# Vegeta2020/SE-SSD

Measured on AMD Instinct MI355X. Metric: KITTI frames/sec (voxelize->backbone->head->NMS), higher is better.
Workload: dtype f32

## Files before the change

### include/sessd_hip.h

```cpp
#ifndef SESSD_HIP_H
#define SESSD_HIP_H

#include <stddef.h>
#include <stdint.h>

#include "sessd_hip_types.h"

#ifdef __cplusplus
extern "C" {
#endif

#define SESSD_OK 0
#define SESSD_EINVAL (-1)
#define SESSD_EWORKSPACE (-2)

typedef void* sessd_stream_t;

const char* sessd_version(void);
int sessd_fill_u32(void* ptr, uint32_t value, size_t n_words, sessd_stream_t stream);
int sessd_fill_u32_multi(int n_segments, void* const* ptrs, const uint32_t* values, const size_t* n_words,
                         sessd_stream_t stream);
void sessd_set_external_clear(int on);
int sessd_stream_create_cu_mask(int n_words, const uint32_t* mask, sessd_stream_t* stream);
int sessd_stream_destroy(sessd_stream_t stream);
// ... 279 lines not shown
                    const float* shift, int relu, const float* residual, void* workspace, size_t workspace_bytes, int workgroups,
                    sessd_stream_t stream);
int sessd_conv2d_sk_active(const float* in, int batch, int cin, int hin, int win, int nclass, const float* const* wpk,
                           const int* ntaps, const int* taps_dy, const int* taps_dx, int in_mul, int tile_h, int tile_w, float* out,
                           int cout, int hout, int wout, int out_mul, const int* out_py, const int* out_px, const float* scale,
                           const float* shift, int relu, const float* residual, const int32_t* tile_list, const int32_t* n_list,
                           int list_cap, int min_rounds, void* workspace, size_t workspace_bytes, int workgroups,
                           sessd_stream_t stream);
int sessd_deconv2d_s2_mfma(const float* in, int batch, int cin, int hin, int win, const float* const* wpk4,
                           const int* ntaps4, const int* taps_dy4, const int* taps_dx4, float* out, int cout,
                           const float* scale, const float* shift, int relu, const float* residual, int tile_cfg,
                           sessd_stream_t stream);
int sessd_deconv2d_s2_mfma_pair(const float* in, int batch, int cin, int hin, int win, const float* const* wpk4_a,
                                const float* const* wpk4_b, const int* ntaps4, const int* taps_dy4, const int* taps_dx4,
                                float* out_a, float* out_b, int cout, const float* scale_a, const float* shift_a,
                                const float* scale_b, const float* shift_b, int relu, const float* residual_a,
                                const float* residual_b, int tile_cfg, sessd_stream_t stream);
int sessd_conv2d_mfma_active(const float* in, int batch, int cin, int hin, int win, const float* wpk, int ntaps, const int* taps_dy,
                             const int* taps_dx, int in_mul, int tile_h, int tile_w, float* out, int cout, int hout, int wout,
                             int out_mul, int out_py, int out_px, const float* scale, const float* shift, int relu,
                             const float* residual, const int32_t* tile_list, const int32_t* n_list, int list_cap, int tile_cfg,
                             sessd_stream_t stream);
int sessd_deconv2d_s2_mfma_pair_active(const float* in, int batch, int cin, int hin, int win, const float* const* wpk4_a,
                                       const float* const* wpk4_b, const int* ntaps4, const int* taps_dy4, const int* taps_dx4,
                                       float* out_a, float* out_b, int cout, const float* scale_a, const float* shift_a,
                                       const float* scale_b, const float* shift_b, int relu, const float* residual_a,
                                       const float* residual_b, const int32_t* tile_list, const int32_t* n_list, int list_cap,
                                       int tile_cfg, sessd_stream_t stream);
int sessd_deconv2d_s2_pair_split_active(const float* in, int batch, int cin, int hin, int win, const void* wsplit_a,
                                        const void* wsplit_b, float* out_a, float* out_b, int cout, const float* scale_a,
                                        const float* shift_a, const float* scale_b, const float* shift_b, int relu,
                                        const float* residual_a, const float* residual_b, const int32_t* tile_list,
                                        const int32_t* n_list, int list_cap, sessd_stream_t stream);
int sessd_ssfa_fuse(const float* x0, const float* x1, const float* w0, const float* w1, float bn_scale0,
                    float bn_shift0, float bn_scale1, float bn_shift1, int batch, int channels, int num_pixels,
                    float* out, sessd_stream_t stream);
int sessd_nchw_split_nhwc(const float* planar, int batch, int channels, int plane, int n_parts, const int* sizes,
                          float* const* parts, sessd_stream_t stream);
int sessd_nhwc_merge_nchw(float* const* parts, int n_parts, const int* sizes, int batch, int channels, int plane, float* planar,
                          sessd_stream_t stream);
size_t sessd_ssfa_fuse_train_workspace_bytes(int batch, int channels, int plane);
int sessd_ssfa_fuse_train_fwd(const float* x0, const float* x1, int batch, int channels, int plane, const float* w0,
                              const float* w1, const float* gamma0, const float* beta0, const float* gamma1, const float* beta1,
                              float eps, float momentum, float* running_mean0, float* running_var0, float* running_mean1,
                              float* running_var1, float* out, float* smap, float* stats, void* workspace,
                              size_t workspace_bytes, sessd_stream_t stream);
int sessd_ssfa_fuse_train_bwd(const float* grad_out, const float* x0, const float* x1, int batch, int channels, int plane,
                              const float* w0, const float* w1, const float* gamma0, const float* beta0, const float* gamma1,
                              const float* beta1, const float* smap, const float* stats, float* dzmap, float* dx0, float* dx1,
                              float* dw0, float* dw1, float* dgamma, float* dbeta, void* workspace, size_t workspace_bytes,
                              sessd_stream_t stream);
int sessd_ssfa_fuse_head(const float* x0, const float* x1, const float* w0, const float* w1, float bn_scale0, float bn_shift0,
                         float bn_scale1, float bn_shift1, int batch, int channels, int num_pixels, float* out,
                         const float* head_w, const float* head_b, int nout, float* head_out, sessd_stream_t stream);
int sessd_ssfa_fuse_head_keys(const float* x0, const float* x1, const float* w0, const float* w1, float bn_scale0,
                              float bn_shift0, float bn_scale1, float bn_shift1, int batch, int channels, int num_pixels,
                              float* out, const float* head_w, const float* head_b, int nout, float* head_out,
                              float score_thresh, unsigned long long* keys, int key_cap, int32_t* key_count,
                              sessd_stream_t stream);
int sessd_ssfa_fuse_head_tasks(const float* x0, const float* x1, const float* w0, const float* w1, float bn_scale0,
                               float bn_shift0, float bn_scale1, float bn_shift1, int batch, int channels, int num_pixels,
                               float* out, const float* head_w, const float* head_b, int num_tasks, float* head_out,
                               float score_thresh, unsigned long long* keys, int key_cap, int32_t* key_count,
                               sessd_stream_t stream);
int sessd_rpn_up_head_tasks(const float* x, const float* up_w, const float* up_scale, const float* up_shift, int batch,
                            int channels, int num_pixels, float* out, const float* head_w, const float* head_b, int num_tasks,
// ... 53 lines not shown
```

### se-ssd_amd/sessd_hip/_lib.py

```python
import ctypes as C
import os

import torch

_HERE = os.path.dirname(os.path.abspath(__file__))
LIB_PATH = os.path.join(os.path.dirname(_HERE), "lib", "libsessd_hip.so")

vp, i32, u32, f32, sz, i64, f64 = C.c_void_p, C.c_int, C.c_uint32, C.c_float, C.c_size_t, C.c_longlong, C.c_double



class ChainLevel(C.Structure):
    _fields_ = [("ksize", i32 * 3), ("stride", i32 * 3), ("pad", i32 * 3), ("out_dims", i32 * 3), ("cap", i32),
                ("indices", vp), ("n_dev", vp)]


class RulebookJob(C.Structure):
    _fields_ = [("in_level", i32), ("out_level", i32), ("ksize", i32 * 3), ("stride", i32 * 3), ("pad", i32 * 3),
                ("nbr", vp), ("tile_mask", vp), ("site_mask", vp), ("perm", vp), ("tile_mask_sorted", vp)]


class FillTilesJob(C.Structure):
    _fields_ = [("out", vp), ("value", vp), ("tile_mask", vp), ("cout", i32), ("h", i32), ("w", i32), ("mask_th", i32), ("tile", i32),
                ("near_kind", i32), ("near_mask", vp)]
# ... 59 lines not shown
    "sessd_boxes_pairwise": (i32, [i32, vp, i32, vp, i32, vp, vp]),
    "sessd_boxes_aligned_overlap_bev": (i32, [vp, vp, i32, vp, vp]),
    "sessd_rotate_iou_eval": (i32, [vp, i32, vp, i32, i32, vp, vp]),
    "sessd_box3d_overlap_eval": (i32, [vp, i32, vp, i32, i32, i32, f64, vp, vp]),
    "sessd_kitti_statistics": (i32, [vp, vp, vp, vp, vp, vp, vp, vp, vp, vp, i32, i32, f64, vp, i32, i32, i32, vp, vp, vp, vp]),
    "sessd_kitti_reduce": (i32, [vp, i32, i32, vp, vp]),
    "sessd_kitti_thresholds": (i32, [vp, i32, i32, i32, vp, vp, vp]),
    "sessd_nms_workspace_bytes": (sz, [i32]),
    "sessd_nms_sorted": (i32, [i32, vp, i32, f32, vp, vp, vp, sz, vp]),
    "sessd_nms_axis_eps_sorted": (i32, [vp, i32, i32, f32, f32, vp, vp, vp, sz, vp]),
    "sessd_conv2d_mfma": (i32, [vp, i32, i32, i32, i32, vp, i32, vp, vp, i32, i32, i32, vp, i32, i32, i32, i32, i32, i32,
                                vp, vp, i32, vp, i32, vp]),
    "sessd_conv3x3_winograd": (i32, [vp, i32, i32, i32, i32, vp, vp, i32, vp, vp, i32, vp, i32, vp]),
    "sessd_conv2d_pack_taps": (i32, [vp, i64, i64, vp, i32, i32, i32, vp, vp]),
    "sessd_conv3x3_winograd_pack": (i32, [vp, i64, i64, i32, i32, i32, i32, vp, vp]),
    "sessd_conv3x3_winograd_sk_workspace_bytes": (sz, [i32, i32, i32, i32, i32, i32]),
    "sessd_conv3x3_winograd_sk_sets": (i32, [vp, i32, i32, i32, i32, i32, vp, vp, i32, vp, vp, i32, vp, vp, sz, i32, i32, vp]),
    "sessd_conv3x3_winograd_sk": (i32, [vp, i32, i32, i32, i32, vp, vp, i32, vp, vp, i32, vp, vp, sz, i32, i32, vp]),
    "sessd_conv3x3_winograd_sk_active": (i32, [vp, i32, i32, i32, i32, vp, vp, i32, vp, vp, i32, vp, vp, vp, i32, i32, vp, sz, i32, i32, vp]),
    "sessd_bev_tile_activity_workspace_bytes": (sz, [i32, i32]),
    "sessd_bev_tile_activity": (i32, [vp, vp, i32, i32, i32, i32, vp, i32, vp, vp, vp, i32, vp, sz, vp]),
    "sessd_fill_inactive_tiles": (i32, [vp, i32, i32, vp]),
    "sessd_conv2d_sk_workspace_bytes": (sz, [i32, i32, i32, i32, i32, i32]),
    "sessd_conv2d_sk_pack": (i32, [vp, i64, i64, vp, i32, i32, i32, vp, vp]),
    "sessd_conv2d_sk": (i32, [vp, i32, i32, i32, i32, i32, vp, vp, vp, vp, i32, i32, i32, vp, i32, i32, i32, i32, vp, vp, vp, vp,
                              i32, vp, vp, sz, i32, vp]),
    "sessd_conv2d_sk_active": (i32, [vp, i32, i32, i32, i32, i32, vp, vp, vp, vp, i32, i32, i32, vp, i32, i32, i32, i32, vp, vp, vp, vp,
                                     i32, vp, vp, vp, i32, i32, vp, sz, i32, vp]),
    "sessd_conv2d_mfma_active": (i32, [vp, i32, i32, i32, i32, vp, i32, vp, vp, i32, i32, i32, vp, i32, i32, i32, i32, i32, i32, vp, vp, i32, vp,
                                       vp, vp, i32, i32, vp]),
    "sessd_deconv2d_s2_mfma_pair_active": (i32, [vp, i32, i32, i32, i32, vp, vp, vp, vp, vp, vp, vp, i32, vp, vp, vp, vp, i32, vp, vp, vp, vp,
                                                 i32, i32, vp]),
    "sessd_deconv2d_s2_pair_split_active": (i32, [vp, i32, i32, i32, i32, vp, vp, vp, vp, i32, vp, vp, vp, vp, i32, vp, vp, vp, vp, i32, vp]),
    "sessd_deconv2d_s2_mfma_pair": (i32, [vp, i32, i32, i32, i32, vp, vp, vp, vp, vp, vp, vp, i32, vp, vp, vp, vp, i32, vp, vp, i32, vp]),
    "sessd_deconv2d_s2_mfma": (i32, [vp, i32, i32, i32, i32, vp, vp, vp, vp, vp, i32, vp, vp, i32, vp, i32, vp]),
    "sessd_ssfa_fuse": (i32, [vp, vp, vp, vp, f32, f32, f32, f32, i32, i32, i32, vp, vp]),
    "sessd_ssfa_fuse_head": (i32, [vp, vp, vp, vp, f32, f32, f32, f32, i32, i32, i32, vp, vp, vp, i32, vp, vp]),
    "sessd_predict_workspace_bytes": (sz, [i32, i32, i32, i32]),
    "sessd_predict": (i32, [vp, i32, i32, vp, i32, vp, f32, i32, i32, f32, vp, f32, vp, vp, vp, vp, vp, sz, vp]),
    "sessd_predict_fused": (i32, [vp, i32, i32, vp, i32, vp, f32, i32, i32, f32, vp, f32, vp, vp, vp, vp, vp, vp, vp, vp, i32, vp, vp, sz, vp]),
    "sessd_ssfa_fuse_head_keys": (i32, [vp, vp, vp, vp, f32, f32, f32, f32, i32, i32, i32, vp, vp, vp, i32, vp, f32, vp, i32, vp, vp]),
    "sessd_ssfa_fuse_head_tasks": (i32, [vp, vp, vp, vp, f32, f32, f32, f32, i32, i32, i32, vp, vp, vp, i32, vp, f32, vp, i32, vp, vp]),
    "sessd_rpn_up_head_tasks": (i32, [vp, vp, vp, vp, i32, i32, i32, vp, vp, vp, i32, vp, f32, vp, i32, vp, vp]),
    "sessd_predict_tasks_workspace_bytes": (sz, [i32, i32, i32, i32, i32]),
    "sessd_predict_tasks": (i32, [vp, i32, i32, i32, vp, i32, vp, f32, i32, i32, f32, vp, f32, vp, vp, vp, vp, vp, vp, vp, vp, vp, i32, vp, vp,
                                  sz, vp]),
    "sessd_predict_di_workspace_bytes": (sz, [i32, i32, i32, i32, i32]),
    "sessd_predict_di": (i32, [vp, i32, i32, i32, vp, i32, vp, f32, i32, i32, f32, vp, f32, vp, vp, vp, vp, vp, vp, vp, vp, vp, i32, vp, vp,
                               vp, vp, vp, vp, vp, sz, vp]),
    "sessd_di_nms_workspace_bytes": (sz, [i32]),
    "sessd_di_nms": (i32, [vp, vp, vp, i32, vp, vp, vp, vp, vp, i32, f32, vp, i32, vp, f32, i32, vp, vp, vp, vp, vp, vp, vp, sz, vp]),
    "sessd_pack_detections": (i32, [vp, vp, vp, vp, i32, i32, vp, vp, i32, vp, vp]),
    "sessd_quads_pairwise": (i32, [i32, vp, i32, vp, i32, vp, f32, vp, vp]),
    "sessd_rotate_nms_workspace_bytes": (sz, [i32]),
    "sessd_rotate_nms_sorted": (i32, [vp, i32, f32, i32, vp, vp, vp, sz, vp]),
    "sessd_rotate_nms_corners_sorted": (i32, [vp, i32, f32, i32, vp, vp, vp, sz, vp]),
    "sessd_sparse_hash_build": (i32, [vp, vp, i32, vp, vp, vp, u32, vp]),
    "sessd_sparse_downsample_workspace_bytes": (sz, [i32, i32, u32]),
    "sessd_sparse_downsample_sites": (i32, [vp, vp, i32, vp, vp, vp, vp, vp, vp, u32, vp, i32, vp, vp, vp, sz, vp]),
    "sessd_sparse_rulebook": (i32, [vp, vp, i32, vp, vp, vp, vp, vp, u32, vp, vp, vp, vp]),
    "sessd_sparse_rulebook_pair": (i32, [vp, vp, i32, vp, vp, vp, vp, vp, u32, vp, vp, vp, vp, vp, vp, vp, vp, u32, vp, vp, vp, vp]),
    "sessd_sparse_downsample_sites_unordered": (i32, [vp, vp, i32, vp, vp, vp, vp, vp, vp, u32, vp, i32, vp, vp, vp]),
    "sessd_sparse_to_dense": (i32, [vp, vp, i32, i32, vp, vp, vp]),
    "sessd_dense_to_sparse": (i32, [vp, vp, i32, i32, vp, vp, vp]),
    "sessd_sparse_to_dense_dev": (i32, [vp, vp, i32, vp, i32, vp, vp, vp]),
    "sessd_dense_to_sparse_dev": (i32, [vp, vp, i32, vp, i32, vp, vp, vp]),
# ... 76 lines not shown
```

### se-ssd_amd/sessd_hip/engine.py

```python
import math
import os

import numpy as np
import torch

from ._lib import lib, check
from . import ops


def _round_up(v, m):
    return (int(v) + m - 1) // m * m


def fold_bn(bn):
    w = bn.weight.detach().float() if bn.weight is not None else torch.ones_like(bn.running_mean)
    b = bn.bias.detach().float() if bn.bias is not None else torch.zeros_like(bn.running_mean)
    scale = w / torch.sqrt(bn.running_var.detach().float() + bn.eps)
    shift = b - bn.running_mean.detach().float() * scale
    return scale.contiguous(), shift.contiguous()


WINO_SPLIT = os.environ.get("SESSD_WINO_SPLIT", "1") != "0"
WINO_LIST_SHAPES = (0, 1, 3) if WINO_SPLIT else (0, 1)
DECONV_SPLIT = os.environ.get("SESSD_DECONV_SPLIT", "1") != "0"
PAIR_SPLIT_CFG = 45

SPMIDDLE_LAYERS = [
    ("subm", 4, 16, 3, 1, 0, "subm0"), ("subm", 16, 16, 3, 1, 0, "subm0"),
    ("conv", 16, 32, 3, 2, 1, None),
    ("subm", 32, 32, 3, 1, 0, "subm1"), ("subm", 32, 32, 3, 1, 0, "subm1"),
    ("conv", 32, 64, 3, 2, 1, None),
    ("subm", 64, 64, 3, 1, 0, "subm2"), ("subm", 64, 64, 3, 1, 0, "subm2"), ("subm", 64, 64, 3, 1, 0, "subm2"),
    ("conv", 64, 64, 3, 2, [0, 1, 1], None),
    ("subm", 64, 64, 3, 1, 0, "subm3"), ("subm", 64, 64, 3, 1, 0, "subm3"), ("subm", 64, 64, 3, 1, 0, "subm3"),
    ("conv", 64, 64, (3, 1, 1), (2, 1, 1), 0, None),
]


def _t3(v):
    return [int(v)] * 3 if isinstance(v, int) else [int(x) for x in v]


class SparsePlan:

    def __init__(self, convs, bns, layers, device):
        self.layers = []
        for (kind, cin, cout, ks, st, pd, key), conv, bn in zip(layers, convs, bns):
            w = conv.weight.detach().to(device=device, dtype=torch.float32).contiguous()
            assert tuple(w.shape[-2:]) == (cin, cout), (w.shape, cin, cout)
            scale, shift = fold_bn(bn)
            self.layers.append(dict(kind=kind, cin=cin, cout=cout, ks=_t3(ks), st=_t3(st), pd=_t3(pd), key=key,
                                    wpk=ops.sparse_pack_weight(w), scale=scale.to(device), shift=shift.to(device)))


def active_tile_constants(neck):
    b0, b1 = neck.bottom_up_block_0, neck.bottom_up_block_1
    def step(seq, ci, bi, c):
        s_, t_ = fold_bn(seq[bi])
# ... 449 lines not shown
        for l in ids:
            if l in (self.ACTIVE_PAIR, self.ACTIVE_CONV):
                for o, v in zip(self.ACTIVE_SLOTS[l][3], self.dn.act_const[l]):
                    outs.append(o); vals.append(v); slots.append(self.ACTIVE_MASK[l]); tiles.append(4 if l == self.ACTIVE_PAIR else 6)
                    near.append(None); kinds.append(0)
                continue
            nr, kind = None, 0
            if self.near_fill:
                rd = self.NEAR_READER.get(l)
                if rd is not None and rd in ids and rd not in self.ACTIVE_SK:
                    nr = self.ACTIVE_MASK[rd]
                elif self.form != "ssfa":
                    pass
                elif self.coarse_fill and l == 2 and 3 in ids and 6 in ids:
                    nr, kind = self.ACTIVE_MASK[3], 2
                elif self.coarse_fill and l == 6 and self.ACTIVE_PAIR in ids:
                    nr, kind = self.ACTIVE_MASK[self.ACTIVE_PAIR], 1
                elif self.coarse_fill and l == 5 and 7 in ids:
                    continue
            outs.append(self.ACTIVE_SLOTS[l][3]); vals.append(self.dn.act_const[l]); slots.append(self.ACTIVE_MASK[l]); tiles.append(2)
            near.append(nr); kinds.append(kind)
        return outs, vals, slots, tiles, near, kinds

    def _active_layers(self):
        if self.ta is None or self._tuning is not None or self.sk_ws is None:
            return []
        return sorted(self.active_cfg)

    def _conv(self, x, layer, out, relu=True, residual=None, name=None, active=None):
        pc, scale, shift = layer
        if active is not None:
            shape, min_rounds = self.active_cfg[active]
            m = self.ACTIVE_MASK[active]
            if active in self.ACTIVE_SK and shape != 30:
                call = lambda: ops.conv2d_mfma_active(x, pc, scale, shift, relu, out, self.ta.tile_list[m], self.ta.n_list[m:m + 1],
                                                      tile_cfg=shape, residual=residual)
            elif active in self.ACTIVE_SK:
                call = lambda: ops.conv2d_sk_active(x, pc, scale, shift, relu, out, self.sk_ws, self.ta.tile_list[m],
                                                    self.ta.n_list[m:m + 1], workgroups=self._wgs(2), residual=residual,
                                                    min_rounds=min_rounds)
            else:
                call = lambda: ops.conv2d_winograd_sk_active(x, pc.upk_sk(shape), pc.cout, scale, shift, relu, out, shape, self.sk_ws,
                                                             self.ta.tile_list[m], self.ta.n_list[m:m + 1],
                                                             workgroups=self._wgs(shape), residual=residual, min_rounds=min_rounds)
            if self._kmarks is not None:
                e0, e1 = torch.cuda.Event(enable_timing=True), torch.cuda.Event(enable_timing=True)
                e0.record()
                r = call()
                e1.record()
                self._kmarks.append((name, e0, e1))
                return r
            return call()
        if self._tuning is not None:
            self._tuning.append((name, x, layer, out, relu, residual))
        if self._kmarks is not None:
            e0, e1 = torch.cuda.Event(enable_timing=True), torch.cuda.Event(enable_timing=True)
            e0.record()
            r = ops.conv2d(x, pc, scale, shift, relu, residual, out, self.tile_cfg.get(name), workspace=self.sk_ws, workgroups=self._wgs_cfg(self.tile_cfg.get(name)))
            e1.record()
            self._kmarks.append((name, e0, e1))
            return r
        return ops.conv2d(x, pc, scale, shift, relu, residual, out, self.tile_cfg.get(name), workspace=self.sk_ws, workgroups=self._wgs_cfg(self.tile_cfg.get(name)))

    def adopt_tuning(self, other):
        self.tile_cfg = dict(other.tile_cfg)
        self.active_cfg = dict(other.active_cfg) if self.ta is not None else {}
        self.sparse_split = dict(other.sparse_split)
        self.sparse_sorted = dict(other.sparse_sorted)
        self.sk_workgroups = other.sk_workgroups
        self.cu_budget = other.cu_budget
        self.merge_branch_convs = other.merge_branch_convs
        self.sk_ws = torch.zeros_like(other.sk_ws) if other.sk_ws is not None else None

    DEFAULT_ACTIVE_CFG = {0: (1, 4), 1: (0, 1), 2: (1, 2), 3: (30, 4), 4: (1, 2), 5: (0, 1), 6: (11, 0), 7: (30, 8), 8: (4, 0), 9: (0, 8)}
    if WINO_SPLIT:
        DEFAULT_ACTIVE_CFG = {l: ((3, mr) if shape == 0 else (shape, mr)) for l, (shape, mr) in DEFAULT_ACTIVE_CFG.items()}

    def force_active_tiles(self, active_cfg=None):
        if self.ta is None:
            raise RuntimeError("this engine has no tile-activity program (active_tiles=False or an unsupported BEV size)")
        if self.form == "rpn":
            self.tile_cfg.update({"blk0.%d" % i: 22 for i in range(len(self.dn.layers))})
            self._need_sk_ws(max(int(lib.sessd_conv3x3_winograd_sk_workspace_bytes(self.B, self.H, self.W, 128, sh, 0)) for sh in (0, 1)))
            cfg = dict(self.DEFAULT_ACTIVE_CFG if active_cfg is None else active_cfg)
            for l, (shape, mr) in cfg.items():
                if l not in self.ACTIVE_SLOTS:
                    raise ValueError("an RPN engine's list layers are %s, got %r" % (sorted(self.ACTIVE_SLOTS), l))
                if self.ACTIVE_SLOTS[l][1][0].upk_sk(shape) is None:
                    raise ValueError("active-tile layer %s: no stream-K Winograd packing for shape %d" % (self.ACTIVE_SLOTS[l][0], shape))
            self.active_cfg = cfg
            return self.active_cfg
        self.tile_cfg.update({"b0.0": 22, "b0.1": 22, "b0.2": 23, "b1.0": 30, "b1.1": 23, "b1.2": 22, "trans_0": 30, "trans_1": 30,
                              "conv_0": 22, "conv_1": 22})
        B = self.B
        self._need_sk_ws(max([int(lib.sessd_conv3x3_winograd_sk_workspace_bytes(2 * B, self.H, self.W, 256, sh, 0)) for sh in (0, 1)] +
                             [int(lib.sessd_conv2d_sk_workspace_bytes(B, self.H, self.W, 256, 1, 0))]))
        cfg = dict(self.DEFAULT_ACTIVE_CFG if active_cfg is None else active_cfg)
        for l, (shape, mr) in cfg.items():
            if l == self.ACTIVE_PAIR and shape == PAIR_SPLIT_CFG and any(pc.wsplit() is None for pc, _, _ in self.ACTIVE_SLOTS[l][1]):
                raise ValueError("active-tile layer %s: no split weight planes (cin %% 16)" % self.ACTIVE_SLOTS[l][0])
            if l in self.ACTIVE_SK or l == self.ACTIVE_PAIR:
                continue
            layers = self.ACTIVE_SLOTS[l][1] if l == self.ACTIVE_CONV else (self.ACTIVE_SLOTS[l][1],)
            if any(pc.upk_sk(shape) is None for pc, _, _ in layers):
                raise ValueError("active-tile layer %s: no stream-K Winograd packing for shape %d" % (self.ACTIVE_SLOTS[l][0], shape))
        self.active_cfg = cfg
        return self.active_cfg

    def autotune(self, candidates=(1, 2, 3, 4, 6, 11, 12), reps=5):
        self._tuning, self._tuning_sparse = [], []
        self.enqueue()
        torch.cuda.synchronize()
        todo, self._tuning = self._tuning, None
        todo_sp, self._tuning_sparse = self._tuning_sparse, None
        st = torch.cuda.current_stream().cuda_stream
        for idx, lay, in_feat, nbr, tm, out_li, out_feat in todo_sp:
            best = (None, 1e30)
            cands = [(a, b, c) for c in ((0, 1) if self.allow_offset_split else (0,)) for a in (1, 2, 4) for b in (2, 3, 4)]
            cands += [(a, 2, 2) for a in (1, 2, 4)]
            if self.levels[out_li]["cap"] >= 65536 or getattr(self, "sparse_mt_candidates", False):
                cands += [(a, b, c) for c in (16, 32) for a in (1, 2, 4) for b in (2, 3)]
            for split, depth, ks in cands:
                if (lay["cout"] // 16) % split or (ks == 1 and depth == 4):
                    continue
                for srt in ((True, False) if self.chain.sort_tiles else (False,)):
                    self.sparse_split[idx] = split + 256 * depth + 65536 * ks
                    self.sparse_sorted[idx] = srt
                    for _ in range(2):
                        self._sconv(lay, in_feat, nbr, tm, out_li, out_feat, st, idx=idx)
                    e0, e1 = torch.cuda.Event(enable_timing=True), torch.cuda.Event(enable_timing=True)
                    e0.record()
                    for _ in range(reps):
                        self._sconv(lay, in_feat, nbr, tm, out_li, out_feat, st, idx=idx)
                    e1.record()
                    torch.cuda.synchronize()
                    t = e0.elapsed_time(e1) / reps
# ... 108 lines not shown
                    dense_t = self.tune_report.get("conv_0", (None, 0.0))[1] + self.tune_report.get("conv_1", (None, 0.0))[1]
                for shape in WINO_LIST_SHAPES:
                    if p0.upk_sk(shape) is None or p1.upk_sk(shape) is None:
                        continue
                    self._need_sk_ws(int(lib.sessd_conv3x3_winograd_sk_workspace_bytes(self.B, self.H, self.W, p0.cout, shape, 0)))
                    for mr in (4, 8, 16, -1):
                        def both(shape=shape, mr=mr):
                            for (pc_, sc_, sh_), xi, xo in ((layer[0], x_in[0], x_out[0]), (layer[1], x_in[1], x_out[1])):
                                ops.conv2d_winograd_sk_active(xi, pc_.upk_sk(shape), pc_.cout, sc_, sh_, True, xo, shape, self.sk_ws,
                                                              self.ta.tile_list[m], self.ta.n_list[m:m + 1], workgroups=self._wgs(shape), min_rounds=mr)
                        tt = timed(both)
                        if tt < best[1]:
                            best = ((shape, mr), tt)
                special_dense[l] = dense_t
                if best[0] is not None and best[1] < dense_t:
                    pick[l] = best
                    gain += dense_t - best[1]
                continue
            pc, scale, shift = layer
            if l in self.ACTIVE_SK:
                if pc.launches[0].ntaps == 1 and pc.cin % 8 == 0:
                    for cfg in (3, 4, 11, 12):
                        tt = timed(lambda: ops.conv2d_mfma_active(x_in, pc, scale, shift, True, x_out, self.ta.tile_list[m],
                                                                  self.ta.n_list[m:m + 1], tile_cfg=cfg))
                        if tt < best[1]:
                            best = ((cfg, 0), tt)
                if pc.sk_args() is not None:
                    self._need_sk_ws(int(lib.sessd_conv2d_sk_workspace_bytes(self.B, *pc.tile_hw(*x_in.shape[2:]), pc.cout, len(pc.launches), 0)))
                    for mr in (1, 4, 8, 16):
                        tt = timed(lambda: ops.conv2d_sk_active(x_in, pc, scale, shift, True, x_out, self.sk_ws, self.ta.tile_list[m],
                                                                self.ta.n_list[m:m + 1], workgroups=self._wgs(2), min_rounds=mr))
                        if tt < best[1]:
                            best = ((30, mr), tt)
            else:
                for shape in WINO_LIST_SHAPES:
                    if pc.upk_sk(shape) is None:
                        continue
                    self._need_sk_ws(int(lib.sessd_conv3x3_winograd_sk_workspace_bytes(self.B, x_in.shape[2], x_in.shape[3], pc.cout, shape, 0)))
                    for mr in self.list_share_candidates:
                        tt = timed(lambda: ops.conv2d_winograd_sk_active(x_in, pc.upk_sk(shape), pc.cout, scale, shift, True, x_out, shape,
                                                                         self.sk_ws, self.ta.tile_list[m], self.ta.n_list[m:m + 1],
                                                                         workgroups=self._wgs(shape), min_rounds=mr))
                        if tt < best[1]:
                            best = ((shape, mr), tt)
            dense_t = self.tune_report.get(name, (None, 0.0))[1]
            if best[0] is not None and best[1] < dense_t:
                pick[l] = best
                gain += dense_t - best[1]
        def overhead(ids):
            fj = self._fill_jobs(ids)
            return timed(lambda: (self.ta.run(L4["indices"], L4["n"], L4["cap"]), self.ta.fill(fj[0], fj[1], layers=fj[2], tiles=fj[3], near=fj[4], near_kind=fj[5])),
                         4 * reps)
        sl = sorted(pick)
        over = overhead(sl) if pick else 0.0
        for l in (self.ACTIVE_CONV, self.ACTIVE_PAIR, 7, 6):
            if l in pick and len(pick) > 1:
                rest = [q for q in sl if q != l]
                over_wo = overhead(rest)
                g = (special_dense[l] if l in special_dense else
                     self.tune_report.get(self.ACTIVE_SLOTS[l][0], (None, 0.0))[1] if l != self.ACTIVE_PAIR else pair_dense_t) - pick[l][1]
                if over - over_wo >= g:
                    del pick[l]
                    sl, over, gain = rest, over_wo, gain - g
        if pick and gain > over:
            self.active_cfg = {l: pick[l][0] for l in pick}
        self.tune_report["active_tiles"] = ({self.ACTIVE_SLOTS[l][0]: v for l, v in self.active_cfg.items()}, gain - over, over,
# ... 436 lines not shown
```

### se-ssd_amd/sessd_hip/ops.py

```python
import ctypes
import os

import torch

from ._lib import lib, check, SessdError


def _stream():
    return torch.cuda.current_stream().cuda_stream


def _p(t):
    return 0 if t is None else t.data_ptr()


def _addr(arr):
    return ctypes.cast(arr, ctypes.c_void_p).value


def _req(t, dtype, name):
    if not t.is_cuda:
        raise ValueError("%s must be a CUDA (HIP) tensor: the SE-SSD hot path has no CPU fallback" % name)
    if t.dtype != dtype:
        raise TypeError("%s must be %s, got %s" % (name, dtype, t.dtype))
# ... 1356 lines not shown
    ws = torch.empty(int(lib.sessd_sparse_conv_wgrad_workspace_bytes(kv, cin, cout)), dtype=torch.uint8, device=in_feat.device)
    check(lib.sessd_sparse_conv_wgrad(in_feat.data_ptr(), cin, grad_out.data_ptr(), cout, nbr.data_ptr(), tile_mask.data_ptr(),
                                      kv, n_out_dev.data_ptr(), cap, gw.data_ptr(), ws.data_ptr(), ws.numel(), _stream()),
          "sparse_conv_wgrad")
    return gw


class Launch:
    __slots__ = ("dy", "dx", "in_mul", "out_mul", "py", "px", "ntaps", "view", "_wpk", "_owner")

    def __init__(self, dy, dx, in_mul, out_mul, py, px, view):
        self.dy, self.dx, self.in_mul, self.out_mul, self.py, self.px, self.view = dy, dx, in_mul, out_mul, py, px, view
        self.ntaps = len(view[3])
        self._wpk = self._owner = None

    @property
    def wpk(self):
        if self._wpk is None:
            pc = self._owner
            self._wpk = pc._make(lambda: _pack_taps_view(*self.view, pc.cout, pc.cin))
        return self._wpk


class PackedConv:

    def __init__(self, launches, cin, cout, kind, stride, w3=None, wt=None):
        self.launches = launches
        self.cin, self.cout, self.kind, self.stride = cin, cout, kind, stride
        self._w3, self._wt = w3, wt
        self._upk = None
        self._upk_sk = [None, None, None, None]
        self._sk = None
        self._wsplit = None
        self._registry = None
        for la in launches:
            la._owner = self
        self.wpk4 = self.ntaps4 = self.dy4 = self.dx4 = None
        if wt is not None:
            self.wpk4 = (ctypes.c_void_p * 4)(*[la.wpk.data_ptr() for la in launches])
            self.ntaps4 = torch.tensor([la.ntaps for la in launches], dtype=torch.int32)
            self.dy4 = torch.zeros((4, 4), dtype=torch.int32)
            self.dx4 = torch.zeros((4, 4), dtype=torch.int32)
            for c, la in enumerate(launches):
                self.dy4[c, :la.ntaps] = la.dy
                self.dx4[c, :la.ntaps] = la.dx

    def _make(self, make):
        return self._registry.create(make) if self._registry is not None else make()

    def out_hw(self, H, W):
        s = self.stride
        return ((H + s - 1) // s, (W + s - 1) // s) if self.kind == "conv" else (s * H, s * W)

    def tile_hw(self, H, W):
        return self.out_hw(H, W) if self.kind == "conv" else (H, W)

    @property
    def is_3x3_s1(self):
        return self._w3 is not None

    @property
    def upk(self):
        if self._upk is None and self.is_3x3_s1 and self.cin % 8 == 0:
            self._upk = self._make(lambda: pack_winograd(self._w3[0], adjoint=self._w3[1]))
        return self._upk

    def upk_sk(self, shape):
        if self._upk_sk[shape] is None and self.is_3x3_s1 and self.cin % (16, 8, 16, 16)[shape] == 0:
            self._upk_sk[shape] = self._make(lambda: pack_winograd_sk(self._w3[0], shape, adjoint=self._w3[1]))
        return self._upk_sk[shape]

    def wsplit(self):
        if self._wt is None or self.cin % 16:
            return None
        if self._registry is not None:
            return pack_deconv2d_s2_split(self._wt)
        if self._wsplit is None:
            self._wsplit = pack_deconv2d_s2_split(self._wt)
        return self._wsplit

    def sk_args(self):
        if self._sk is None:
            n = len(self.launches)
            if self.cin % 16 or n > 4:
                return None
            ncg = (self.cout + 127) // 128
            wpk, dy, dx = [], (ctypes.c_int * (9 * n))(), (ctypes.c_int * (9 * n))()
            for c, la in enumerate(self.launches):
                w, so, sc, taps = la.view
                nt = len(taps)
                out = torch.empty((ncg, self.cin // 16, nt, 2048), dtype=torch.float32, device=w.device)
                check(lib.sessd_conv2d_sk_pack(w.data_ptr(), int(so), int(sc), (ctypes.c_int * nt)(*[int(t) for t in taps]), nt,
                                               self.cout, self.cin, out.data_ptr(), _stream()), "conv2d_sk_pack")
                wpk.append(out)
                for t in range(nt):
                    dy[9 * c + t], dx[9 * c + t] = int(la.dy[t]), int(la.dx[t])
            self._sk = dict(wpk=wpk, wptr=(ctypes.c_void_p * n)(*[t.data_ptr() for t in wpk]),
                            ntaps=(ctypes.c_int * n)(*[la.ntaps for la in self.launches]), dy=dy, dx=dx,
                            py=(ctypes.c_int * n)(*[la.py for la in self.launches]),
                            px=(ctypes.c_int * n)(*[la.px for la in self.launches]), n=n)
        return self._sk


def _pack_taps_view(w, out_stride, in_stride, tap_offsets, cout, cin):
    _req(w, torch.float32, "weight")
    nt = len(tap_offsets)
    cp = (cout + 31) // 32 * 32
    out = torch.empty((cin // 2, nt, 2, cp), dtype=torch.float32, device=w.device)
    check(lib.sessd_conv2d_pack_taps(w.data_ptr(), int(out_stride), int(in_stride), (ctypes.c_int * nt)(*[int(t) for t in tap_offsets]),
                                     nt, cout, cin, out.data_ptr(), _stream()), "conv2d_pack_taps")
    _repack_note("dense", w=w, out=out, so=int(out_stride), sc=int(in_stride), taps=[int(t) for t in tap_offsets], cout=int(cout),
                 cin=int(cin), kind=0, flip=0, layout=0)
# ... 244 lines not shown

DECONV_SPLIT_TAPS = ((1, 1), (1, 2), (2, 1), (2, 2), (1, 0), (2, 0), (0, 1), (0, 2), (0, 0))


def pack_deconv2d_s2_split(weight):
    w = weight.detach().to(torch.float32)
    ci, co, kh, kw = w.shape
    if kh != 3 or kw != 3 or ci % 16:
        raise ValueError("pack_deconv2d_s2_split: a (Cin, Cout, 3, 3) weight with Cin % 16 == 0")
    ng = (co + 127) // 128
    wt = torch.zeros((9, ci, ng * 128), dtype=torch.float32, device=w.device)
    for t, (ky, kx) in enumerate(DECONV_SPLIT_TAPS):
        wt[t, :, :co] = w[:, :, ky, kx]
    planes = []
    for _ in range(3):
        p = wt.to(torch.bfloat16)
        planes.append(p)
        wt = wt - p.to(torch.float32)
    pl = torch.stack(planes).view(3, 9, ci // 16, 2, 8, ng, 4, 32)
    return pl.permute(5, 2, 1, 0, 6, 3, 7, 4).contiguous().view(ng, ci // 16, 9, 3, 4, 64, 8)


def deconv2d_s2_pair_split_active(x, pc_a, pc_b, scale_a, shift_a, scale_b, shift_b, relu, out_a, out_b, tile_list, n_list, residual_a=None,
                                  residual_b=None):
    _req(tile_list, torch.int32, "tile_list"); _req(n_list, torch.int32, "n_list")
    wa, wb = pc_a.wsplit(), pc_b.wsplit()
    if wa is None or wb is None:
        raise ValueError("deconv2d_s2_pair_split_active needs cin % 16 == 0")
    args = _pair_args(x, pc_a, pc_b, (wa.data_ptr(), wb.data_ptr()), scale_a, shift_a, scale_b, shift_b, relu, out_a, out_b, residual_a,
                      residual_b)
    check(lib.sessd_deconv2d_s2_pair_split_active(*args, tile_list.data_ptr(), n_list.data_ptr(), tile_list.numel(), _stream()),
          "deconv2d_s2_pair_split_active")
    return out_a, out_b


def pack_deconv2d_ks(weight, s):
    w = weight.detach().to(torch.float32).contiguous()
    ci, co, kh, kw = w.shape
    s = int(s)
    assert s >= 2 and kh == s and kw == s and ci % 2 == 0
    zero = torch.zeros(1, dtype=torch.int32)
    launches = []
    for py in range(s):
        for px in range(s):
            launches.append(Launch(zero, zero, 1, s, py, px, (w, s * s, co * s * s, [py * s + px])))
    pc = PackedConv(launches, ci, co, "deconv_ks", s)
    for la in launches:
        la.wpk
    return pc


class PackedDeconvKs:

    def __init__(self, wpk, cin, cout, s):
        self.wpk, self.cin, self.cout, self.stride, self.kind = wpk, cin, cout, s, "deconv_ks_slice"


def pack_deconv_ks_slice(weight, s):
    w = weight.detach().to(torch.float32).contiguous()
    _req(w, torch.float32, "weight")
    ci, co, kh, kw = w.shape
    s = int(s)
    if s not in (1, 2, 4) or kh != s or kw != s:
        raise ValueError("pack_deconv_ks_slice: kernel size = stride in {1, 2, 4} expected, got kernel %dx%d, s = %d" % (kh, kw, s))
    if ci % 2 or co % 32:
        raise ValueError("pack_deconv_ks_slice: even cin and cout %% 32 == 0 expected, got %d -> %d" % (ci, co))
# ... 700 lines not shown
```

Before: 2236.

## Add bf16x3-split MFMA kernel for active-tile 3x3 stride-2 conv

Adds a new HIP kernel for the active-tile 3x3 stride-2 BEV conv. It splits f32 activations and weights into three bf16 planes and accumulates the cross terms with 32x32x16 bf16 MFMA, using double-buffered LDS and a pipeline tuned with scheduling barriers. The autotuner now times this path against the existing stream-K and MFMA variants and selects it only when it is fastest. The bf16x3 split aims for near-f32 accuracy through bf16 matrix cores, at the cost of extra MFMAs and a separate weight packing.

Result: faster. 2284 (median of 6 runs) (+2.1%).

```diff
diff --git a/include/sessd_hip.h b/include/sessd_hip.h
--- a/include/sessd_hip.h
+++ b/include/sessd_hip.h
@@ -335,6 +335,9 @@
                                         const float* shift_a, const float* scale_b, const float* shift_b, int relu,
                                         const float* residual_a, const float* residual_b, const int32_t* tile_list,
                                         const int32_t* n_list, int list_cap, sessd_stream_t stream);
+int sessd_conv2d_s2_split_active(const float* in, int batch, int cin, int hin, int win, const void* wsplit, float* out, int cout,
+                                 int hout, int wout, const float* scale, const float* shift, int relu, const float* residual,
+                                 const int32_t* tile_list, const int32_t* n_list, int list_cap, sessd_stream_t stream);
 int sessd_ssfa_fuse(const float* x0, const float* x1, const float* w0, const float* w1, float bn_scale0,
                     float bn_shift0, float bn_scale1, float bn_shift1, int batch, int channels, int num_pixels,
                     float* out, sessd_stream_t stream);
diff --git a/se-ssd_amd/csrc/dense_conv_s2_split.hip b/se-ssd_amd/csrc/dense_conv_s2_split.hip
--- /dev/null
+++ b/se-ssd_amd/csrc/dense_conv_s2_split.hip
@@ -0,0 +1,273 @@
+#include "common.hpp"
+#include "bf16_split.hpp"
+
+namespace {
+
+using f32x16 = __attribute__((ext_vector_type(16))) float;
+typedef unsigned int u32x2g __attribute__((__vector_size__(8)));
+typedef unsigned int u32x4g __attribute__((__vector_size__(16)));
+typedef __bf16 bf16x8 __attribute__((ext_vector_type(8)));
+using sessd::split3_pk;
+
+typedef __amdgpu_buffer_rsrc_t rsrc_t;
+__device__ __forceinline__ rsrc_t make_rsrc(const void* base, unsigned bytes) {
+  return __builtin_amdgcn_make_buffer_rsrc(const_cast<void*>(base), (short)0, (int)bytes, 0x00020000);
+}
+__device__ __forceinline__ float bufload(rsrc_t rsrc, unsigned voff, unsigned soff) {
+  return __builtin_bit_cast(float, __builtin_amdgcn_raw_buffer_load_b32(rsrc, (int)voff, (int)soff, 0));
+}
+#define SESSD_OOB 0x80000000u
+#define SESSD_LDS_BARRIER() asm volatile("s_waitcnt lgkmcnt(0)\n\ts_barrier" ::: "memory")
+
+struct ConvS2SplitArgs {
+  const float* in;
+  const void* w;
+  float* out;
+  const float* scale;
+  const float* shift;
+  const float* residual;
+  const int* tile_list;
+  const int* n_list;
+  int list_cap, batch, cin, hin, win, cout, hout, wout, relu, ngroups;
+};
+
+__device__ __forceinline__ bool tile_of(const ConvS2SplitArgs& A, int n_list, int k, int& img, int& y0, int& x0) {
+  const int ntiles2 = (A.hout >> 1) * (A.wout >> 1), tw2 = A.wout >> 1;
+  const int ent = k < n_list ? A.tile_list[k] : -1;
+  const bool live = ent >= 0 && ent < A.batch * ntiles2;
+  img = live ? ent / ntiles2 : 0;
+  const int t = live ? ent - img * ntiles2 : 0;
+  y0 = 2 * (t / tw2);
+  x0 = 2 * (t - (t / tw2) * tw2);
+  return live;
+}
+
+constexpr int XBUF = 3 * 2 * 3 * 256;
+
+__global__ __launch_bounds__(256, 2) void conv_s2_split_kernel(ConvS2SplitArgs A) {
+  __shared__ __attribute__((aligned(16))) unsigned lds[2 * XBUF];
+  const int tid = threadIdx.x, lane = tid & 63, wave = tid >> 6;
+  const int j = lane & 31, h = lane >> 5;
+  const int n_list = __builtin_amdgcn_readfirstlane(min(A.n_list[0], A.list_cap));
+  const int unit = blockIdx.x / A.ngroups, grp = blockIdx.x - unit * A.ngroups;
+  if (unit * 16 >= n_list) return;
+
+  const int npix = A.hin * A.win;
+  const unsigned plane4 = (unsigned)npix * 4u;
+  const int KS = A.cin >> 4;
+  const rsrc_t xr = make_rsrc(A.in, (unsigned)A.batch * A.cin * plane4);
+  const rsrc_t wr = make_rsrc(A.w, (unsigned)A.ngroups * KS * (27u * 4096u));
+
+  const int spb = wave & 1, sq = wave >> 1;
+  unsigned xo[3][3];
+  {
+    int img, y0, x0;
+    const bool live = tile_of(A, n_list, unit * 16 + spb * 8 + (j >> 2), img, y0, x0);
+    const int iy0 = 2 * (y0 + ((j >> 1) & 1)) - 1, ix0 = 2 * (x0 + (j & 1)) - 1;
+    const unsigned base = (unsigned)(img * A.cin + h * 8 + sq * 4) * (unsigned)npix;
+#pragma unroll
+    for (int ky = 0; ky < 3; ++ky)
+#pragma unroll
+      for (int kx = 0; kx < 3; ++kx) {
+        const int iy = iy0 + ky, ix = ix0 + kx;
+        xo[ky][kx] = (live && iy >= 0 && iy < A.hin && ix >= 0 && ix < A.win) ? (base + (unsigned)(iy * A.win + ix)) * 4u : SESSD_OOB;
+      }
+  }
+  const int wthr = (spb * 3 * 64 + lane) * 4 + sq * 2;
+  float xs[3][4];
+#define SESSD_CS_LOADX(KSTEP, KY)                                                                   \
+  {                                                                                                 \
+    const unsigned c0 = (unsigned)min((KSTEP), KS - 1) * 16u;                                       \
+    _Pragma("unroll") for (int kx = 0; kx < 3; ++kx)                                                \
+      _Pragma("unroll") for (int i = 0; i < 4; ++i)                                                 \
+        xs[kx][i] = bufload(xr, xo[KY][kx], (c0 + i) * plane4);                                     \
+  }
+#define SESSD_CS_SPLIT_STORE(VOFF)                                                                  \
+  {                                                                                                 \
+    _Pragma("unroll") for (int kx = 0; kx < 3; ++kx) {                                              \
+      u32x2g t0, t1, t2;                                                                            \
+      _Pragma("unroll") for (int q = 0; q < 2; ++q) {                                               \
+        unsigned a0, a1, a2;                                                                        \
+        split3_pk(xs[kx][2 * q], xs[kx][2 * q + 1], a0, a1, a2);                                    \
+        t0[q] = a0; t1[q] = a1; t2[q] = a2;                                                         \
+      }                                                                                             \
+      unsigned* dst = lds + (VOFF) + wthr + kx * (2 * 3 * 256);                                     \
+      *static_cast<u32x2g*>(__builtin_assume_aligned(dst, 8)) = t0;                                 \
+      *static_cast<u32x2g*>(__builtin_assume_aligned(dst + 256, 8)) = t1;                           \
+      *static_cast<u32x2g*>(__builtin_assume_aligned(dst + 512, 8)) = t2;                           \
+    }                                                                                               \
+  }
+
+  const int cb = wave;
+  const int rthr = lane * 4;
+  const unsigned wvo = (unsigned)(cb * 1024 + lane * 16);
+  const unsigned wgrp = (unsigned)grp * (unsigned)KS * (27u * 4096u);
+  const int tlast = KS * 9 - 1;
+  f32x16 acc[2], accl[2], tot[2];
+  const f32x16 zero16 = {0.f, 0.f, 0.f, 0.f, 0.f, 0.f, 0.f, 0.f, 0.f, 0.f, 0.f, 0.f, 0.f, 0.f, 0.f, 0.f};
+#pragma unroll
+  for (int q = 0; q < 2; ++q) acc[q] = accl[q] = tot[q] = zero16;
+  bf16x8 af[3][3], bf[2][2][3];
+
+#define SESSD_CS_LOADA(SET, TG)                                                                     \
+  {                                                                                                 \
+    const unsigned ws = wgrp + (unsigned)min((TG), tlast) * (3u * 4096u);                           \
+    _Pragma("unroll") for (int p = 0; p < 3; ++p)                                                   \
+      af[SET][p] = __builtin_bit_cast(bf16x8, __builtin_amdgcn_raw_buffer_load_b128(wr, (int)wvo, (int)(ws + 4096u * p), 0)); \
+  }
+#define SESSD_CS_READB(VOFF, KX, BS)                                                                \
+  {                                                                                                 \
+    _Pragma("unroll") for (int q = 0; q < 2; ++q)                                                   \
+      _Pragma("unroll") for (int p = 0; p < 3; ++p)                                                 \
+        bf[BS][q][p] = __builtin_bit_cast(bf16x8, *static_cast<const u32x4g*>(__builtin_assume_aligned( \
+            lds + (VOFF) + rthr + (((KX)*2 + q) * 3 + p) * 256, 16)));                              \
+  }
+#define SESSD_CS_M(ACC, KX, BS, PA, PB)                                                             \
+  _Pragma("unroll") for (int q = 0; q < 2; ++q)                                                     \
+    ACC[q] = __builtin_amdgcn_mfma_f32_32x32x16_bf16(af[KX][PA], bf[BS][q][PB], ACC[q], 0, 0, 0);
+#define SESSD_CS_MSMALL(KX, BS)                                                                     \
+  SESSD_CS_M(accl, KX, BS, 2, 0)                                                                    \
+  SESSD_CS_M(accl, KX, BS, 1, 1)                                                                    \
+  SESSD_CS_M(accl, KX, BS, 0, 2)                                                                    \
+  SESSD_CS_M(accl, KX, BS, 1, 0)                                                                    \
+  SESSD_CS_M(accl, KX, BS, 0, 1)
+#define SESSD_CS_MMA(KX, BS)                                                                        \
+  {                                                                                                 \
+    SESSD_CS_MSMALL(KX, BS)                                                                         \
+    SESSD_CS_M(acc, KX, BS, 0, 0)                                                                   \
+  }
+#define SESSD_CS_MMA_FIRST(BS)                                                                      \
+  {                                                                                                 \
+    _Pragma("unroll") for (int q = 0; q < 2; ++q) tot[q] += acc[q];                                 \
+    SESSD_CS_MSMALL(0, BS)                                                                          \
+    _Pragma("unroll") for (int q = 0; q < 2; ++q)                                                   \
+      acc[q] = __builtin_amdgcn_mfma_f32_32x32x16_bf16(af[0][0], bf[BS][q][0], zero16, 0, 0, 0);    \
+  }
+#define SESSD_CS_STEP(KS_, KY, S0, S1)                                                              \
+  {                                                                                                 \
+    const int tg = (KS_)*9 + (KY)*3;                                                                \
+    SESSD_CS_READB(voff, 1, S1)                                                                     \
+    SESSD_CS_LOADA(2, tg + 2)                                                                       \
+    __builtin_amdgcn_sched_barrier(0);                                                              \
+    SESSD_CS_MMA_FIRST(S0)                                                                          \
+    SESSD_CS_SPLIT_STORE(voff ^ XBUF)                                                               \
+    _Pragma("unroll") for (int g = 0; g < 12; ++g) {                                                \
+      __builtin_amdgcn_sched_group_barrier(0x008, 1, 0);                                            \
+      __builtin_amdgcn_sched_group_barrier(0x002, 9, 0);                                            \
+    }                                                                                               \
+    __builtin_amdgcn_sched_barrier(0);                                                              \
+    SESSD_CS_READB(voff, 2, S0)                                                                     \
+    SESSD_CS_LOADX((KS_) + ((KY) + 2) / 3, ((KY) + 2) % 3)                                          \
+    SESSD_CS_LOADA(0, tg + 3)                                                                       \
+    __builtin_amdgcn_sched_barrier(0);                                                              \
+    SESSD_CS_MMA(1, S1)                                                                             \
+    __builtin_amdgcn_sched_barrier(0);                                                              \
+    SESSD_LDS_BARRIER();                                                                            \
+    voff ^= XBUF;                                                                                   \
+    SESSD_CS_READB(voff, 0, S1)                                                                     \
+    SESSD_CS_LOADA(1, tg + 4)                                                                       \
+    __builtin_amdgcn_sched_barrier(0);                                                              \
+    SESSD_CS_MMA(2, S0)                                                                             \
+    __builtin_amdgcn_sched_barrier(0);                                                              \
+  }
+
+  int voff = 0;
+  SESSD_CS_LOADX(0, 0)
+  SESSD_CS_LOADA(0, 0)
+  SESSD_CS_LOADA(1, 1)
+  __builtin_amdgcn_sched_barrier(0);
+  SESSD_CS_SPLIT_STORE(0)
+  SESSD_CS_LOADX(0, 1)
+  SESSD_LDS_BARRIER();
+  SESSD_CS_READB(0, 0, 0)
+  __builtin_amdgcn_sched_barrier(0);
+  int ks = 0;
+  for (; ks + 1 < KS; ks += 2) {
+    SESSD_CS_STEP(ks, 0, 0, 1)
+    SESSD_CS_STEP(ks, 1, 1, 0)
+    SESSD_CS_STEP(ks, 2, 0, 1)
+    SESSD_CS_STEP(ks + 1, 0, 1, 0)
+    SESSD_CS_STEP(ks + 1, 1, 0, 1)
+    SESSD_CS_STEP(ks + 1, 2, 1, 0)
+  }
+  if (ks < KS) {
+    SESSD_CS_STEP(ks, 0, 0, 1)
+    SESSD_CS_STEP(ks, 1, 1, 0)
+    SESSD_CS_STEP(ks, 2, 0, 1)
+  }
+#undef SESSD_CS_LOADX
+#undef SESSD_CS_SPLIT_STORE
+#undef SESSD_CS_LOADA
+#undef SESSD_CS_READB
+#undef SESSD_CS_M
+#undef SESSD_CS_MMA
+#undef SESSD_CS_MSMALL
+#undef SESSD_CS_MMA_FIRST
+#undef SESSD_CS_STEP
+
+  const unsigned oplane = (unsigned)(A.hout * A.wout);
+  const unsigned obytes = (unsigned)A.batch * A.cout * oplane * 4u;
+  const float* res = A.residual;
+  const rsrc_t orr = make_rsrc(A.out, obytes);
+  const rsrc_t rr = make_rsrc(res ? res : A.out, res ? obytes : 0u);
+  const rsrc_t scr = make_rsrc(A.scale ? A.scale : A.in, A.scale ? (unsigned)A.cout * 4u : 0u);
+  const rsrc_t shr = make_rsrc(A.shift ? A.shift : A.in, A.shift ? (unsigned)A.cout * 4u : 0u);
+  const int co0 = grp * 128 + cb * 32 + 4 * h;
+  float scv[16], shv[16];
+#pragma unroll
+  for (int r = 0; r < 16; ++r) {
+    const int k = (r & 3) + 8 * (r >> 2);
+    scv[r] = A.scale ? bufload(scr, (unsigned)(co0 + k) * 4u, 0) : 1.f;
+    shv[r] = bufload(shr, (unsigned)(co0 + k) * 4u, 0);
+  }
+#pragma unroll
+  for (int q = 0; q < 2; ++q) {
+    int img, y0, x0;
+    const bool live = tile_of(A, n_list, unit * 16 + q * 8 + (j >> 2), img, y0, x0);
+    const int y = y0 + ((j >> 1) & 1), x = x0 + (j & 1);
+    const unsigned vbase = ((unsigned)(img * A.cout + co0) * oplane + (unsigned)(y * A.wout + x)) * 4u;
+    unsigned vo[16];
+    float rv[16];
+#pragma unroll
+    for (int r = 0; r < 16; ++r) {
+      const int k = (r & 3) + 8 * (r >> 2);
+      vo[r] = (live && co0 + k < A.cout) ? vbase + (unsigned)k * oplane * 4u : SESSD_OOB;
+      rv[r] = bufload(rr, vo[r], 0);
+    }
+#pragma unroll
+    for (int r = 0; r < 16; ++r) {
+      float v = fmaf((tot[q][r] + acc[q][r]) + accl[q][r], scv[r], shv[r]);
+      if (A.relu) v = fmaxf(v, 0.f);
+      if (res) v += rv[r];
+      __builtin_amdgcn_raw_buffer_store_b32(__builtin_bit_cast(unsigned, v), orr, (int)vo[r], 0, 0);
+    }
+  }
+}
+
+size_t split_pack_bytes(int cin, int cout) { return (size_t)sessd_divup(cout, 128) * (cin / 16) * 27 * 4096; }
+
+}
+
+extern "C" {
+
+int sessd_conv2d_s2_split_active(const float* in, int batch, int cin, int hin, int win, const void* wsplit, float* out, int cout,
+                                 int hout, int wout, const float* scale, const float* shift, int relu, const float* residual,
+                                 const int32_t* tile_list, const int32_t* n_list, int list_cap, hipStream_t stream) {
+  if (cin < 16 || cin % 16 || batch < 1 || cout < 1 || hout < 2 || wout < 2 || (hout & 1) || (wout & 1)) return SESSD_EINVAL;
+  if ((hin != 2 * hout && hin != 2 * hout - 1) || (win != 2 * wout && win != 2 * wout - 1)) return SESSD_EINVAL;
+  if (!in || !wsplit || !out || !tile_list || !n_list || list_cap < 1) return SESSD_EINVAL;
+  if ((long long)batch * cout * hout * wout * 4 >= 0x7fffffffLL || (long long)batch * cin * hin * win * 4 >= 0x7fffffffLL) return SESSD_EINVAL;
+  if (split_pack_bytes(cin, cout) >= 0x7fffffffULL) return SESSD_EINVAL;
+  ConvS2SplitArgs A;
+  A.in = in; A.w = wsplit; A.out = out; A.scale = scale; A.shift = shift; A.residual = residual;
+  A.tile_list = tile_list; A.n_list = n_list; A.list_cap = list_cap;
+  A.batch = batch; A.cin = cin; A.hin = hin; A.win = win; A.cout = cout; A.hout = hout; A.wout = wout; A.relu = relu;
+  A.ngroups = sessd_divup(cout, 128);
+  const long long wgs = (long long)sessd_divup(list_cap, 16) * A.ngroups;
+  if (wgs > 0x7fffffffLL) return SESSD_EINVAL;
+  SESSD_LAUNCH(conv_s2_split_kernel, dim3((unsigned)wgs), dim3(256), 0, stream, A);
+  SESSD_CHECK_LAUNCH();
+  return SESSD_OK;
+}
+
+}
diff --git a/se-ssd_amd/sessd_hip/_lib.py b/se-ssd_amd/sessd_hip/_lib.py
--- a/se-ssd_amd/sessd_hip/_lib.py
+++ b/se-ssd_amd/sessd_hip/_lib.py
@@ -115,6 +115,7 @@
     "sessd_deconv2d_s2_mfma_pair_active": (i32, [vp, i32, i32, i32, i32, vp, vp, vp, vp, vp, vp, vp, i32, vp, vp, vp, vp, i32, vp, vp, vp, vp,
                                                  i32, i32, vp]),
     "sessd_deconv2d_s2_pair_split_active": (i32, [vp, i32, i32, i32, i32, vp, vp, vp, vp, i32, vp, vp, vp, vp, i32, vp, vp, vp, vp, i32, vp]),
+    "sessd_conv2d_s2_split_active": (i32, [vp, i32, i32, i32, i32, vp, vp, i32, i32, i32, vp, vp, i32, vp, vp, vp, i32, vp]),
     "sessd_deconv2d_s2_mfma_pair": (i32, [vp, i32, i32, i32, i32, vp, vp, vp, vp, vp, vp, vp, i32, vp, vp, vp, vp, i32, vp, vp, i32, vp]),
     "sessd_deconv2d_s2_mfma": (i32, [vp, i32, i32, i32, i32, vp, vp, vp, vp, vp, i32, vp, vp, i32, vp, i32, vp]),
     "sessd_ssfa_fuse": (i32, [vp, vp, vp, vp, f32, f32, f32, f32, i32, i32, i32, vp, vp]),
diff --git a/se-ssd_amd/sessd_hip/engine.py b/se-ssd_amd/sessd_hip/engine.py
--- a/se-ssd_amd/sessd_hip/engine.py
+++ b/se-ssd_amd/sessd_hip/engine.py
@@ -24,6 +24,8 @@
 WINO_LIST_SHAPES = (0, 1, 3) if WINO_SPLIT else (0, 1)
 DECONV_SPLIT = os.environ.get("SESSD_DECONV_SPLIT", "1") != "0"
 PAIR_SPLIT_CFG = 45
+CONV_S2_SPLIT = os.environ.get("SESSD_CONV_S2_SPLIT", "1") != "0"
+S2_SPLIT_CFG = 46
 
 SPMIDDLE_LAYERS = [
     ("subm", 4, 16, 3, 1, 0, "subm0"), ("subm", 16, 16, 3, 1, 0, "subm0"),
@@ -539,7 +541,10 @@
         if active is not None:
             shape, min_rounds = self.active_cfg[active]
             m = self.ACTIVE_MASK[active]
-            if active in self.ACTIVE_SK and shape != 30:
+            if active in self.ACTIVE_SK and shape == S2_SPLIT_CFG:
+                call = lambda: ops.conv2d_s2_split_active(x, pc, scale, shift, relu, out, self.ta.tile_list[m], self.ta.n_list[m:m + 1],
+                                                          residual=residual)
+            elif active in self.ACTIVE_SK and shape != 30:
                 call = lambda: ops.conv2d_mfma_active(x, pc, scale, shift, relu, out, self.ta.tile_list[m], self.ta.n_list[m:m + 1],
                                                       tile_cfg=shape, residual=residual)
             elif active in self.ACTIVE_SK:
@@ -606,9 +611,11 @@
         for l, (shape, mr) in cfg.items():
             if l == self.ACTIVE_PAIR and shape == PAIR_SPLIT_CFG and any(pc.wsplit() is None for pc, _, _ in self.ACTIVE_SLOTS[l][1]):
                 raise ValueError("active-tile layer %s: no split weight planes (cin %% 16)" % self.ACTIVE_SLOTS[l][0])
+            if shape == S2_SPLIT_CFG and (l not in self.ACTIVE_SK or self.ACTIVE_SLOTS[l][1][0].wsplit_s2() is None):
+                raise ValueError("active-tile layer %s: no split weight planes of a 3x3 stride-2 conv (cin %% 16)" % self.ACTIVE_SLOTS[l][0])
             if l in self.ACTIVE_SK or l == self.ACTIVE_PAIR:
                 continue
-            layers = self.ACTIVE_SLOTS[l][1] if l == self.ACTIVE_CONV else (self.ACTIVE_SLOTS[l][1],)
+            layers =self.ACTIVE_SLOTS[l][1] if l == self.ACTIVE_CONV else (self.ACTIVE_SLOTS[l][1],)
             if any(pc.upk_sk(shape) is None for pc, _, _ in layers):
                 raise ValueError("active-tile layer %s: no stream-K Winograd packing for shape %d" % (self.ACTIVE_SLOTS[l][0], shape))
         self.active_cfg = cfg
@@ -783,6 +790,11 @@
                                                                 self.ta.n_list[m:m + 1], workgroups=self._wgs(2), min_rounds=mr))
                         if tt < best[1]:
                             best = ((30, mr), tt)
+                if CONV_S2_SPLIT and pc.wsplit_s2() is not None:
+                    tt = timed(lambda: ops.conv2d_s2_split_active(x_in, pc, scale, shift, True, x_out, self.ta.tile_list[m],
+                                                                  self.ta.n_list[m:m + 1]))
+                    if tt < best[1]:
+                        best = ((S2_SPLIT_CFG, 0), tt)
             else:
                 for shape in WINO_LIST_SHAPES:
                     if pc.upk_sk(shape) is None:
diff --git a/se-ssd_amd/sessd_hip/ops.py b/se-ssd_amd/sessd_hip/ops.py
--- a/se-ssd_amd/sessd_hip/ops.py
+++ b/se-ssd_amd/sessd_hip/ops.py
@@ -1412,6 +1412,7 @@
         self._upk_sk = [None, None, None, None]
         self._sk = None
         self._wsplit = None
+        self._wsplit_s2 = None
         self._registry = None
         for la in launches:
             la._owner = self
@@ -1458,6 +1459,16 @@
         if self._wsplit is None:
             self._wsplit = pack_deconv2d_s2_split(self._wt)
         return self._wsplit
+
+    def wsplit_s2(self):
+        if self.kind != "conv" or self.stride != 2 or self.launches[0].ntaps != 9 or self.cin % 16:
+            return None
+        w = self.launches[0].view[0]
+        if self._registry is not None:
+            return pack_conv2d_s2_split(w)
+        if self._wsplit_s2 is None:
+            self._wsplit_s2 = pack_conv2d_s2_split(w)
+        return self._wsplit_s2
 
     def sk_args(self):
         if self._sk is None:
@@ -1768,6 +1779,38 @@
     check(lib.sessd_deconv2d_s2_pair_split_active(*args, tile_list.data_ptr(), n_list.data_ptr(), tile_list.numel(), _stream()),
           "deconv2d_s2_pair_split_active")
     return out_a, out_b
+
+
+def pack_conv2d_s2_split(weight):
+    w = weight.detach().to(torch.float32)
+    if w.dim() != 4 or w.shape[2] != 3 or w.shape[3] != 3 or w.shape[1] % 16:
+        raise ValueError("pack_conv2d_s2_split: a (Cout, Cin, 3, 3) weight with Cin % 16 == 0")
+    co, ci = w.shape[0], w.shape[1]
+    ng = (co + 127) // 128
+    wt = torch.zeros((9, ci, ng * 128), dtype=torch.float32, device=w.device)
+    wt[:, :, :co] = w.permute(2, 3, 1, 0).reshape(9, ci, co)
+    planes = []
+    for _ in range(3):
+        p = wt.to(torch.bfloat16)
+        planes.append(p)
+        wt = wt - p.to(torch.float32)
+    pl = torch.stack(planes).view(3, 9, ci // 16, 2, 8, ng, 4, 32)
+    return pl.permute(5, 2, 1, 0, 6, 3, 7, 4).contiguous().view(ng, ci // 16, 9, 3, 4, 64, 8)
+
+
+def conv2d_s2_split_active(x, pc, scale, shift, relu, out, tile_list, n_list, residual=None):
+    _req(x, torch.float32, "x"); _req(out, torch.float32, "out"); _req(tile_list, torch.int32, "tile_list"); _req(n_list, torch.int32, "n_list")
+    ws = pc.wsplit_s2()
+    if ws is None:
+        raise ValueError("conv2d_s2_split_active needs a 3x3 stride-2 conv with cin % 16 == 0")
+    B, ci, H, W = x.shape
+    ho, wo = pc.out_hw(H, W)
+    if ci != pc.cin or tuple(out.shape) != (B, pc.cout, ho, wo):
+        raise ValueError("conv2d_s2_split_active: x (B, cin, H, W) and out (B, cout, ceil(H/2), ceil(W/2))")
+    check(lib.sessd_conv2d_s2_split_active(x.data_ptr(), B, ci, H, W, ws.data_ptr(), out.data_ptr(), pc.cout, ho, wo, _p(scale), _p(shift),
+                                           1 if relu else 0, _p(residual), tile_list.data_ptr(), n_list.data_ptr(), tile_list.numel(),
+                                           _stream()), "conv2d_s2_split_active")
+    return out
 
 
 def pack_deconv2d_ks(weight, s):
```
